# matteobutano/optimal_crowds

Hardware: NVIDIA B200
Metric: hjb_gcell_updates_per_s (higher is better)
Workload: dtype f64

## Files before the change

### optimal_crowds_b200/csrc/oc_hjb.cu

```cuda
#include <cmath>
#include <algorithm>
#include <vector>

#include "oc_common.h"
#include "oc_hjb_fused.cuh"
#include "oc_hjb_final.h"
#include "oc_rk45.h"
#include "oc_vels.h"

namespace {

constexpr int TX = 128, TY = 16, NTHREADS = 256;
constexpr int SW = TX + 2;

struct Comb {
    const double *y;
    const double *k[6];
    double a[6];
    double h;
};

template <int N>
__device__ __forceinline__ double comb_eval(const Comb &c, size_t idx) {
    if (N == 0) return c.y[idx];
// ... 233 lines not shown
    size_t pool_used = 0;
    cudaEvent_t get_event() {
        if (pool_used == pool.size()) { cudaEvent_t e; cudaEventCreate(&e); pool.push_back(e); }
        return pool[pool_used++];
    }
    void begin(int cls, double bytes) {
        if (!profile) return;
        Rec r{cls, bytes, get_event(), get_event()};
        cudaEventRecord(r.a, st);
        recs.push_back(r);
    }
    void end() {
        if (!profile) return;
        cudaEventRecord(recs.back().b, st);
    }
    void collect(oc_hjb_stats *out) {
        for (auto &r : recs) {
            float ms = 0;
            cudaEventElapsedTime(&ms, r.a, r.b);
            out->cls_launches[r.cls]++;
            out->cls_ms[r.cls] += ms;
            out->cls_bytes[r.cls] += r.bytes;
        }
        for (auto e : pool) cudaEventDestroy(e);
        pool.clear(); recs.clear();
    }

    template <int N, int MODE>
    void launch_stage(const Comb &c, double *kout, double *yn, const ErrArgs &ea) {
        dim3 grid(nbx, nby);
        begin(0, 8.0 * (double)n * (MODE == 1 ? 9 : N + 3));
        hjb_stage_kernel<N, MODE><<<grid, NTHREADS, 0, st>>>(c, coef, kout, yn, ea, partial, Ny, Nx, diff_over_dxdy);
        end();
        launches++;
    }
    void stage(int N, const Comb &c, double *kout) {
        ErrArgs ea{};
        switch (N) {
            case 0: launch_stage<0, 0>(c, kout, nullptr, ea); break;
            case 1: launch_stage<1, 0>(c, kout, nullptr, ea); break;
            case 2: launch_stage<2, 0>(c, kout, nullptr, ea); break;
            case 3: launch_stage<3, 0>(c, kout, nullptr, ea); break;
            case 4: launch_stage<4, 0>(c, kout, nullptr, ea); break;
            case 5: launch_stage<5, 0>(c, kout, nullptr, ea); break;
        }
    }
    int fused_rc = 0, fused_gx = 0, fused_gy = 0;
    void fused_plan(int n_sm, int forced_rc = 0) {
        fused_gx = (Nx + fused::VX - 1) / fused::VX;
        fused_rc = forced_rc > 0 ? forced_rc : fused::plan_chunk_rows(Nx, Ny, n_sm, 1, 0);
        fused_gy = (Ny + fused_rc - 1) / fused_rc;
    }
    fused::MapCache maps;
    int launch_fused(int ne, fused::Args &a) {
        fused::set_tensor_maps(a, Ny, &maps);
        dim3 grid(fused_gx, fused_gy);
        begin(0, 8.0 * (double)n * (5 + ne));
        OC_CUDA(fused::launch<false>(ne, a, grid, st));
        end();
        launches++;
        return OC_OK;
    }
    int reduce_to_host(size_t off, double *out, int gx = -1, int gy = -1) {
        if (gx < 0) { gx = nbx; gy = nby; }
        begin(2, 8.0 * ((double)gx * gy + gy));
        rowgroup_sum_kernel<<<gy, NTHREADS, 0, st>>>(partial + off, gx, rowsum_d);
        end();
        launches++;
        OC_CUDA(cudaMemcpyAsync(rowsum_h, rowsum_d, sizeof(double) * gy, cudaMemcpyDeviceToHost, st));
        OC_CUDA(cudaStreamSynchronize(st));
        double s = 0.0;
        for (int i = 0; i < gy; i++) s += rowsum_h[i];
        *out = s;
        return OC_OK;
    }
};

int ensure_ws(oc_ctx *ctx, size_t n, int nbx, int nby) {
    int rc = oc_ensure_buffer(ctx->hjb_ws, ctx->hjb_ws_bytes, 10 * n * sizeof(double), false, "HJB workspace");
    if (rc) return rc;
    size_t np = (size_t)2 * nbx * nby + nby + 64;
    {
        size_t fgx = (size_t)(nbx * TX + fused::VX - 1) / fused::VX + 1, fgy = (size_t)(nby * TY + 15) / 16 + 1;
        np = std::max(np, 2 * fgx * fgy + fgy + 64);
    }
    if ((rc = oc_ensure_buffer(ctx->hjb_partial, ctx->hjb_partial_bytes, np * sizeof(double), false, "HJB partial sums")))
        return rc;
    size_t hp = (size_t)std::max(nby, (nby * TY + 15) / 16 + 1) + 16;
    return oc_ensure_buffer(ctx->h_pinned, ctx->h_pinned_bytes, hp * sizeof(double), true, "pinned host scratch");
}

int ensure_final_reduce(oc_ctx *ctx, int slots) { return ocfinal::ensure(ctx, slots); }
void final_reduce_args(oc_ctx *ctx, int slot, fused::Args &fa) { ocfinal::set_args(ctx, slot, ++ctx->fr_seq, fa); }
inline bool final_ready(oc_ctx *ctx, int slot, unsigned long long seq, double *out) { return ocfinal::ready(ctx, slot, seq, out); }
int wait_final(oc_ctx *ctx, int slot, unsigned long long seq, cudaStream_t st, double *out) {
    return ocfinal::wait(ctx, slot, seq, st, out);
}

}

extern "C" int oc_hjb_rhs(oc_ctx *ctx, const double *d_phi, const double *d_V, const double *d_m,
                          const oc_hjb_params *prm, double *d_out, void *stream) {
    OC_ARG(ctx && d_phi && d_V && prm && d_out, "NULL argument");
    OC_CUDA(cudaSetDevice(ctx->device));
    Solver s{};
    s.ctx = ctx; s.st = (cudaStream_t)stream; s.Ny = ctx->Ny; s.Nx = ctx->Nx;
    s.n = (size_t)s.Ny * s.Nx;
    s.nbx = (s.Nx + TX - 1) / TX; s.nby = (s.Ny + TY - 1) / TY;
    int rc = ensure_ws(ctx, s.n, s.nbx, s.nby);
    if (rc) return rc;
    s.coef = ctx->hjb_ws;
// ... 55 lines not shown
    s.profile = prm->profile != 0;
    OC_CUDA(cudaEventRecord(ctx->ev0, s.st));

    prep_kernel<<<(unsigned)((n + 255) / 256), 256, 0, s.st>>>(d_V, d_m, prm->g, 1.0 / (prm->mu * s2), n, s.coef, s.y);
    s.launches++;
    rk45::Controller ctl(T, t_eval, nt);
    {
        Comb c{};
        c.y = s.y;
        s.stage(0, c, s.K[0]);
        stats->nfev++;
    }
    if (ctl.needs_initial_step()) {
        dim3 grid(s.nbx, s.nby);
        init_norm_kernel<<<grid, NTHREADS, 0, s.st>>>(s.y, s.K[0], nullptr, rtol, atol, s.Ny, s.Nx, s.partial, 0);
        s.launches++;
        double s0, s1, sq2;
        if ((rc = s.reduce_to_host(0, &s0))) return rc;
        if ((rc = s.reduce_to_host((size_t)s.nbx * s.nby, &s1))) return rc;
        const double d1 = std::sqrt(s1) / sqrt_n;
        const double h0 = ctl.initial_h0(std::sqrt(s0) / sqrt_n, d1);
        Comb c{};
        c.y = s.y; c.k[0] = s.K[0]; c.a[0] = 1.0; c.h = h0 * ctl.direction;
        s.stage(1, c, s.K[1]);
        stats->nfev++;
        init_norm_kernel<<<grid, NTHREADS, 0, s.st>>>(s.y, s.K[0], s.K[1], rtol, atol, s.Ny, s.Nx, s.partial, 1);
        s.launches++;
        if ((rc = s.reduce_to_host(0, &sq2))) return rc;
        ctl.set_initial_step(h0, d1, std::sqrt(sq2) / sqrt_n / h0);
    }
    stats->h0 = ctl.h_abs;

    bool use_fused = prm->fused != 0 && s.Ny > fused::HY + 1 && s.Nx > fused::HX + 1, fused_attempt = false;
    double *phi_scratch = nullptr;
    if (use_fused) {
        int n_sm = 148;
        cudaDeviceGetAttribute(&n_sm, cudaDevAttrMultiProcessorCount, ctx->device);
        s.fused_plan(n_sm, prm->chunk_rows);
        size_t np_need = (size_t)2 * s.fused_gx * s.fused_gy + s.fused_gy;
        if (ctx->hjb_partial_bytes < np_need * sizeof(double) || ctx->h_pinned_bytes < ((size_t)s.fused_gy + 16) * sizeof(double)) {
            oc::set_error("internal: fused partial buffers too small");
            return OC_ERR_ARG;
        }
        if (!d_phi && d_vx && d_vy) {
            size_t need = (size_t)fused::NE_MAX * n * sizeof(double);
            if ((rc = oc_ensure_buffer(ctx->hjb_scratch, ctx->hjb_scratch_bytes, need, false, "phi scratch"))) return rc;
            phi_scratch = ctx->hjb_scratch;
        }
    }
    const size_t n_int = (size_t)(s.Ny - 2) * (s.Nx - 2);
    const bool final_in_kernel = use_fused && s.fused_gy <= fused::MAX_FINAL_ROWS;
    if (final_in_kernel && (rc = ensure_final_reduce(ctx, 1))) return rc;
    const bool want_out = d_phi || (d_vx && d_vy);

    while (ctl.begin_step()) {
        bool accepted = false;
        while (!accepted && ctl.propose(prm->forced_h, prm->n_forced_h)) {
            const double h = ctl.h;
            fused_attempt = use_fused && (!want_out || d_phi || ctl.n_emit() <= fused::NE_MAX);
            double se;
            if (fused_attempt) {
                fused::Args fa{};
                fa.y = s.y; fa.k1 = s.K[0]; fa.coef = s.coef; fa.ynew = s.ynew; fa.k7 = s.K[6]; fa.partial = s.partial;
                fa.A = s.diff_over_dxdy; fa.rtol = rtol; fa.atol = atol;
                fa.Ny = s.Ny; fa.Nx = s.Nx; fa.RC = s.fused_rc;
                fa.row_base = 0; fa.own0 = 0; fa.own1 = s.Ny; fa.phi_row_base = 0;
                const int n_emit = want_out ? ctl.n_emit() : 0;
                int e0 = 0;
                do {
                    const int ne = std::min(n_emit - e0, fused::NE_MAX);
                    fused::set_attempt(fa, ctl, e0, ne, d_phi, phi_scratch, n);
                    if (final_in_kernel) final_reduce_args(ctx, 0, fa);
                    if ((rc = s.launch_fused(ne, fa))) return rc;
                    e0 += ne;
                } while (e0 < n_emit);
                stats->nfev += 6;
                if (final_in_kernel) {
                    if ((rc = wait_final(ctx, 0, fa.seq, s.st, &se))) return rc;
                } else if ((rc = s.reduce_to_host(0, &se, s.fused_gx, s.fused_gy))) return rc;
            } else {
            for (int sgi = 1; sgi < 6; sgi++) {
                Comb c{};
                c.y = s.y; c.h = h;
                for (int j = 0; j < sgi; j++) { c.k[j] = s.K[j]; c.a[j] = rk45::A[sgi][j]; }
                s.stage(sgi, c, s.K[sgi]);
            }
            {
                Comb c{};
                c.y = s.y; c.h = h;
                int m = 0;
                for (int j = 0; j < 6; j++)
                    if (j != 1) { c.k[m] = s.K[j]; c.a[m] = rk45::B[j]; m++; }
                ErrArgs ea{};
                for (int j = 0; j < 6; j++) ea.k[j] = s.K[j];
                for (int j = 0; j < 7; j++) ea.e[j] = rk45::E[j];
                ea.h = h; ea.rtol = rtol; ea.atol = atol;
                s.launch_stage<5, 1>(c, s.K[6], s.ynew, ea);
            }
            stats->nfev += 6;
            if ((rc = s.reduce_to_host(0, &se))) return rc;
            }
            const double error_norm = std::sqrt(se) / sqrt_n;
            const int ntr = ctl.attempts();
            if (trace_h && ntr < trace_cap) { trace_h[ntr] = h; trace_err[ntr] = error_norm; }
            accepted = ctl.judge(error_norm);
        }
        if (!accepted) break;

        if (fused_attempt) {
            for (int e = 0; e < ctl.n_emit(); e++) {
                const int kd = ctl.sample_column(e);
                if (d_vx && d_vy && kd >= 1) {
                    const double *ph = fused::sample_slice(ctl, e, d_phi, phi_scratch, n);
                    const int sl = nt - 1 - kd;
                    dim3 grid((s.Nx - 2 + 63) / 64, (s.Ny - 2 + 3) / 4);
                    s.begin(1, 8.0 * (double)n * 3);
                    vels_kernel<<<grid, NTHREADS, 0, s.st>>>(ph, s.Ny, s.Nx, prm->mu, prm->lim, 1.0 / (2 * ctx->dx), 1.0 / (2 * ctx->dy),
                                                             d_vx + (size_t)sl * n_int, d_vy + (size_t)sl * n_int);
                    s.end();
                    s.launches++;
                }
            }
        } else {
            int e = 0;
            while (e < ctl.n_emit()) {
                DenseArgs a{};
                a.yold = s.y;
                for (int j = 0; j < 7; j++) { a.k[j] = s.K[j]; for (int p = 0; p < 4; p++) a.P[j][p] = rk45::P[j][p]; }
                a.h = ctl.h; a.mu = prm->mu; a.lim = prm->lim; a.inv_two_dx = 1.0 / (2 * ctx->dx); a.inv_two_dy = 1.0 / (2 * ctx->dy);
                int m = 0;
                bool any = false;
                for (; m < DMAX && e < ctl.n_emit(); e++) {
                    int kd = ctl.sample_column(e);
                    a.x[m] = ctl.sample_x(e);
                    a.phi[m] = d_phi ? d_phi + (size_t)kd * n : nullptr;
                    int sl = nt - 1 - kd;
                    bool has_v = d_vx && d_vy && kd >= 1;
                    a.vx[m] = has_v ? d_vx + (size_t)sl * n_int : nullptr;
                    a.vy[m] = has_v ? d_vy + (size_t)sl * n_int : nullptr;
                    if (a.phi[m] || a.vx[m]) { any = true; m++; }
                }
                a.n_emit = m;
                if (any) {
                    dim3 grid((s.Nx + DTX - 1) / DTX, (s.Ny + DTY - 1) / DTY);
                    double words = 7.0;
                    for (int q = 0; q < m; q++) words += (a.phi[q] ? 1.0 : 0.0) + (a.vx[q] ? 2.0 : 0.0);
                    s.begin(1, 8.0 * (double)n * words);
                    hjb_dense_kernel<<<grid, NTHREADS, 0, s.st>>>(a, s.Ny, s.Nx);
                    s.end();
                    s.launches++;
                }
            }
        }
        ctl.accept();
        std::swap(s.y, s.ynew);
        std::swap(s.K[0], s.K[6]);
    }
    OC_CUDA(cudaEventRecord(ctx->ev1, s.st));
    OC_CUDA(cudaStreamSynchronize(s.st));
    OC_CUDA(cudaGetLastError());
    float ms = 0;
    OC_CUDA(cudaEventElapsedTime(&ms, ctx->ev0, ctx->ev1));
    stats->gpu_ms = ms;
    s.collect(stats);
    ctl.report(stats);
    stats->launches = s.launches;
    oc::count_launch(s.launches);
    if (trace_n) *trace_n = ctl.attempts();
    if (ctl.status == -1) {
        oc::set_error("RK45: required step size is less than spacing between numbers (t=%g)", ctl.t);
        return OC_ERR_STEP_TOO_SMALL;
    }
    return OC_OK;
}

namespace {

struct BatchRoom {
    Solver s;
    enum Phase { START, INIT0, INIT1, STEP, DONE } phase = START;
    const double *V = nullptr, *m = nullptr;
    double *phi = nullptr, *scratch = nullptr, *vx = nullptr, *vy = nullptr;
    double *rs_d = nullptr, *rs_h = nullptr;
    int rs_stride = 0;
    cudaEvent_t ev = nullptr;
    unsigned long long wait_seq = 0;
    rk45::Controller ctl;
    double g = 0, inv_mu_s2 = 0, mu = 0;
    double h0 = 0, d1 = 0;
    double step_sum = 0.0;
    fused::Args fa{};
    oc_hjb_stats st{};
};

}

extern "C" int oc_hjb_solve_batch(oc_ctx *ctx, int n_rooms, const double *const *d_V, const double *const *d_m,
                                  const oc_hjb_params *prm, double T, const double *t_eval, int nt,
                                  double *const *d_phi, double *const *d_vx, double *const *d_vy,
                                  oc_hjb_stats *stats, void *stream) {
    OC_ARG(prm && n_rooms >= 1, "NULL argument");
    std::vector<oc_hjb_room> same(n_rooms, oc_hjb_room{prm->sigma, prm->mu, prm->g, T, t_eval, nt, 0});
    return oc_hjb_solve_multi(ctx, n_rooms, d_V, d_m, same.data(), prm, d_phi, d_vx, d_vy, stats, stream);
}

extern "C" int oc_hjb_solve_multi(oc_ctx *ctx, int n_rooms, const double *const *d_V, const double *const *d_m,
                                  const oc_hjb_room *spec, const oc_hjb_params *prm, double *const *d_phi,
                                  double *const *d_vx, double *const *d_vy, oc_hjb_stats *stats, void *stream) {
    OC_ARG(ctx && d_V && prm && stats && n_rooms >= 1, "NULL argument");
// ... 281 lines not shown
```

### optimal_crowds_b200/csrc/oc_hjb_fused.cuh

```cuda
#pragma once
#include <cuda.h>
#include <cuda_runtime.h>

#include <cstddef>
#include <cstdint>

#include "oc_rk45.h"

namespace fused {

#ifndef OC_BX
#define OC_BX 128
#endif
#ifndef OC_PF
#define OC_PF 6
#endif
#ifndef OC_PD
#define OC_PD (OC_PF - 1)
#endif
constexpr int BX = OC_BX;
constexpr int HX = 8;
constexpr int VX = BX - 2 * HX;
constexpr int HY = 6;
constexpr int PF = OC_PF;
// ... 40 lines not shown
    double *phi[NE_MAX];
    double ha21;
    double ha3[2], ha4[3], ha5[4], ha6[5];
    double hb[6];
    double he[7];
    double w[NE_MAX][7];
    double A;
    double rtol, atol;
    int Ny, Nx, RC;
    int row_base, own0, own1, phi_row_base;
    unsigned *ticket;
    double *result;
    unsigned long long *result_seq;
    unsigned long long seq;
    double *peer_ynew[2], *peer_k7[2];
    int peer_row_base[2];
    int nranks, my_rank;
    double *peer_inbox[P2P_MAX_RANKS];
};
constexpr int MAX_FINAL_ROWS = 2 * 6 * (BX + 2) - 8;

inline double *sample_slice(const rk45::Controller &c, int e, double *phi, double *scratch, size_t slice) {
    return phi ? phi + (size_t)c.sample_column(e) * slice : scratch + (size_t)(e % NE_MAX) * slice;
}
inline void set_attempt(Args &a, const rk45::Controller &c, int e0, int ne, double *phi, double *scratch, size_t slice) {
    const double h = c.h;
    a.ha21 = h * rk45::A[1][0];
    for (int j = 0; j < 2; j++) a.ha3[j] = h * rk45::A[2][j];
    for (int j = 0; j < 3; j++) a.ha4[j] = h * rk45::A[3][j];
    for (int j = 0; j < 4; j++) a.ha5[j] = h * rk45::A[4][j];
    for (int j = 0; j < 5; j++) a.ha6[j] = h * rk45::A[5][j];
    for (int j = 0; j < 6; j++) a.hb[j] = h * rk45::B[j];
    for (int j = 0; j < 7; j++) a.he[j] = h * rk45::E[j];
    for (int i = 0; i < ne; i++) {
        const double x = c.sample_x(e0 + i);
        const double pw[4] = {x, x * x, x * x * x, x * x * x * x};
        for (int j = 0; j < 7; j++) {
            double acc = 0.0;
            for (int q = 0; q < 4; q++) acc += rk45::P[j][q] * pw[q];
            a.w[i][j] = h * acc;
        }
        a.phi[i] = sample_slice(c, e0 + i, phi, scratch, slice);
    }
}

__device__ __forceinline__ void cp_async8_if(void *smem, const void *gmem, bool ok) {
    unsigned s = (unsigned)__cvta_generic_to_shared(smem);
    asm volatile("{ .reg .pred p; setp.ne.b32 p, %2, 0; @p cp.async.ca.shared.global [%0], [%1], 8; }"
                 ::"r"(s), "l"(gmem), "r"((int)ok) : "memory");
}
__device__ __forceinline__ void st_if(double *p, double v, bool ok) {
    asm volatile("{ .reg .pred p; setp.ne.b32 p, %2, 0; @p st.global.f64 [%0], %1; }" ::"l"(p), "d"(v), "r"((int)ok) : "memory");
}
__device__ __forceinline__ void cp_async_commit() { asm volatile("cp.async.commit_group;" ::: "memory"); }
template <int N>
__device__ __forceinline__ void cp_async_wait() { asm volatile("cp.async.wait_group %0;" ::"n"(N) : "memory"); }

__device__ __forceinline__ void mbar_init(unsigned long long *bar, unsigned count) {
    asm volatile("mbarrier.init.shared::cta.b64 [%0], %1;" ::"r"((unsigned)__cvta_generic_to_shared(bar)), "r"(count) : "memory");
}
__device__ __forceinline__ void mbar_expect_tx(unsigned long long *bar, unsigned bytes) {
    asm volatile("mbarrier.arrive.expect_tx.shared::cta.b64 _, [%0], %1;"
                 ::"r"((unsigned)__cvta_generic_to_shared(bar)), "r"(bytes) : "memory");
}
__device__ __forceinline__ void bulk_g2s(void *smem, const void *gmem, unsigned bytes, unsigned long long *bar) {
    asm volatile("cp.async.bulk.shared::cluster.global.mbarrier::complete_tx::bytes [%0], [%1], %2, [%3];"
                 ::"r"((unsigned)__cvta_generic_to_shared(smem)), "l"(gmem), "r"(bytes),
                   "r"((unsigned)__cvta_generic_to_shared(bar)) : "memory");
}
__device__ __forceinline__ void tma_g2s_2d(unsigned smem, const CUtensorMap *map, int cx, int cy, unsigned bar) {
    asm volatile("cp.async.bulk.tensor.2d.shared::cluster.global.tile.mbarrier::complete_tx::bytes [%0], [%1, {%2, %3}], [%4];"
                 ::"r"(smem), "l"(reinterpret_cast<uint64_t>(map)), "r"(cx), "r"(cy), "r"(bar) : "memory");
}
__device__ __forceinline__ bool elect_one() {
    unsigned pred;
    asm volatile("{ .reg .pred p; elect.sync _|p, 0xffffffff; selp.u32 %0, 1, 0, p; }" : "=r"(pred));
    return pred != 0;
}
__device__ __forceinline__ void mbar_expect_tx_u32(unsigned bar, unsigned bytes) {
    asm volatile("mbarrier.arrive.expect_tx.shared::cta.b64 _, [%0], %1;" ::"r"(bar), "r"(bytes) : "memory");
}
__device__ __forceinline__ void bulk_g2s_u32(unsigned smem, const void *gmem, unsigned bytes, unsigned bar) {
    asm volatile("cp.async.bulk.shared::cluster.global.mbarrier::complete_tx::bytes [%0], [%1], %2, [%3];"
                 ::"r"(smem), "l"(gmem), "r"(bytes), "r"(bar) : "memory");
}
__device__ __forceinline__ void mbar_wait_u32(unsigned bar, unsigned parity) {
    asm volatile(
        "{\n"
        ".reg .pred p;\n"
        "OC_WAITU_%=:\n"
        "mbarrier.try_wait.parity.shared::cta.b64 p, [%0], %1;\n"
        "@p bra OC_DONEU_%=;\n"
        "bra OC_WAITU_%=;\n"
        "OC_DONEU_%=:\n"
        "}\n" ::"r"(bar), "r"(parity) : "memory");
}
__device__ __forceinline__ void mbar_wait(unsigned long long *bar, unsigned parity) {
    asm volatile(
        "{\n"
        ".reg .pred p;\n"
        "OC_WAIT_%=:\n"
        "mbarrier.try_wait.parity.shared::cta.b64 p, [%0], %1;\n"
        "@p bra OC_DONE_%=;\n"
        "bra OC_WAIT_%=;\n"
        "OC_DONE_%=:\n"
        "}\n" ::"r"((unsigned)__cvta_generic_to_shared(bar)), "r"(parity) : "memory");
}

__device__ __forceinline__ double rhs_pre(double up, double lf, double rt, double C, double Aw, double dw) {
    return fma(Aw, (up + lf) + rt, dw * C);
}
__device__ __forceinline__ double rhs_fin(double pre, double dn, double Aw) { return fma(Aw, dn, pre); }

__device__ __forceinline__ double rcp_pos(double x) {
    double r;
    asm("rcp.approx.ftz.f64 %0, %1;" : "=d"(r) : "d"(x));
    double e = fma(-x, r, 1.0);
    r = fma(r, e, r);
    e = fma(-x, r, 1.0);
    r = fma(r, e, r);
    return r;
}

struct __align__(128) Smem {
    double pf[NG][3][GR][BX];
    double2 ex[2][3][BX + 2];
    double cst[(1 + NE_MAX) * 6];
    double red[BX / 32];
    unsigned long long full[NG];
};
static_assert(sizeof(double2) * 2 * 3 * (BX + 2) >= sizeof(double) * MAX_FINAL_ROWS, "final reduction staging");

__device__ __forceinline__ int mirror(int i, int n) { return i < 0 ? -i : (i >= n ? 2 * (n - 1) - i : i); }

template <int NE, bool P2P, bool BULK>
__device__ __forceinline__ void hjb_fused_body(const Args &a) {
    extern __shared__ __align__(128) unsigned char smem_raw[];
    Smem &sm = *reinterpret_cast<Smem *>(smem_raw);
    const int tid = threadIdx.x;
    const int x0 = blockIdx.x * VX - HX;
    const int gx = x0 + tid;
    const int c0 = max(x0, 0), c1 = min(x0 + BX, a.Nx);
    const int gxm = min(max(mirror(gx, a.Nx), c0), c1 - 1);
    const int lt = BULK ? gxm - x0 : tid;
    const int y0 = a.own0 + blockIdx.y * a.RC;
    const int y1 = min(y0 + a.RC, a.own1);
    const bool col_out = tid >= HX && tid < BX - HX && gx < a.Nx;
    const int phi_shift = (a.row_base - a.phi_row_base) * a.Nx;

    for (int i = tid; i < 2 * 3 * (BX + 2); i += BX) (&sm.ex[0][0][0])[i] = make_double2(0.0, 0.0);
    if (tid < 6) {
        const int j = tid == 0 ? 0 : tid + 1;
        sm.cst[tid] = a.he[j];
#pragma unroll
        for (int ee = 0; ee < NE; ee++) sm.cst[6 * (ee + 1) + tid] = a.w[ee][j];
    }
    if (BULK && tid == 0) {
#pragma unroll
        for (int s = 0; s < NG; s++) mbar_init(&sm.full[s], 1);
        asm volatile("fence.mbarrier_init.release.cluster;" ::: "memory");
    }
    __syncthreads();
    unsigned sm_pf = (unsigned)__cvta_generic_to_shared(&sm.pf[0][0][0][0]);
    unsigned sm_full = (unsigned)__cvta_generic_to_shared(&sm.full[0]);
    asm volatile("" : "+r"(sm_pf), "+r"(sm_full));

    double yw[7], k1w[7], Aw[7], dw[7], k2w[5], k3w[7], k4w[7], k5w[7], k6w[7];
    double u2[3], u3[4], u4[5], u5[6], u6[7], un[8];
#pragma unroll
    for (int i = 0; i < 7; i++) { yw[i] = 0; k1w[i] = 0; Aw[i] = 0; dw[i] = 0; k3w[i] = 0; k4w[i] = 0; k5w[i] = 0; k6w[i] = 0; }
#pragma unroll
    for (int i = 0; i < 5; i++) k2w[i] = 0;
    u2[0] = u2[1] = u2[2] = 0; u3[1] = u3[2] = u3[3] = 0; u4[2] = u4[3] = u4[4] = 0;
    u5[3] = u5[4] = u5[5] = 0; u6[4] = u6[5] = u6[6] = 0; un[5] = un[6] = un[7] = 0;

    const int r_begin = y0 - HY, r_end = y1 + HY;
    const unsigned row_bytes = (unsigned)(c1 - c0) * 8u;
    const int warp = __shfl_sync(0xffffffffu, tid >> 5, 0);
    constexpr unsigned TILE_BYTES = 3u * GR * BX * 8u, FIELD_BYTES = GR * BX * 8u, ROW_BYTES = BX * 8u;
    auto issue_group = [&](int ga, int slot) {
        if (warp == 0 && ga < r_end && elect_one()) {
            const unsigned bar = sm_full + 8u * slot, dst = sm_pf + TILE_BYTES * slot;
            if (ga >= 0 && ga + GR <= a.Ny) {
                mbar_expect_tx_u32(bar, TILE_BYTES);
                tma_g2s_2d(dst, &a.tm_y, x0, ga - a.row_base, bar);
                tma_g2s_2d(dst + FIELD_BYTES, &a.tm_k1, x0, ga - a.row_base, bar);
                tma_g2s_2d(dst + 2u * FIELD_BYTES, &a.tm_coef, x0, ga - a.row_base, bar);
            } else {
                mbar_expect_tx_u32(bar, 3u * GR * row_bytes);
#pragma unroll 1
                for (int j = 0; j < GR; j++) {
                    const int rm = min(max(mirror(ga + j, a.Ny), 0), a.Ny - 1);
                    const int g = (rm - a.row_base) * a.Nx + c0;
                    const unsigned d = dst + ROW_BYTES * j + 8u * (c0 - x0);
                    bulk_g2s_u32(d, a.y + g, row_bytes, bar);
                    bulk_g2s_u32(d + FIELD_BYTES, a.k1 + g, row_bytes, bar);
                    bulk_g2s_u32(d + 2u * FIELD_BYTES, a.coef + g, row_bytes, bar);
                }
            }
        }
    };
    auto issue = [&](int row, int slot) {
        const int rm = min(max(mirror(row, a.Ny), 0), a.Ny - 1);
        const int g = (rm - a.row_base) * a.Nx + gxm;
        const bool ok = row < r_end;
        cp_async8_if(&sm.pf[0][0][slot][tid], a.y + g, ok);
        cp_async8_if(&sm.pf[0][1][slot][tid], a.k1 + g, ok);
        cp_async8_if(&sm.pf[0][2][slot][tid], a.coef + g, ok);
        cp_async_commit();
    };

    if (BULK) issue_group(r_begin, 0);
    else {
#pragma unroll 1
        for (int q = 0; q < PD; q++) issue(r_begin + q, q);
    }

    constexpr int NV = NE < OC_VREGCONST ? NE : OC_VREGCONST;
    double wv[NV > 0 ? NV : 1][6], hev[6];
#pragma unroll
    for (int ee = 0; ee < NV; ee++)
#pragma unroll
        for (int j = 0; j < 6; j++) wv[ee][j] = sm.cst[6 * (ee + 1) + j];
#pragma unroll
    for (int j = 0; j < 6; j++) hev[j] = a.he[j == 0 ? 0 : j + 1];
    const double dwall = -4.0 * a.A;

    double acc = 0.0;
    unsigned ph_base = 0;
#pragma unroll 1
    for (int rb = r_begin; rb < r_end; rb += UNROLL) {
#pragma unroll
      for (int uu = 0; uu < UNROLL; uu++) {
        const int r = rb + uu;
        const int s0 = uu % PF;
        const int buf = uu & 1;
        const int gi = uu / GR, gj = uu % GR;
        if (BULK) {
            if (gj == 0) {
                issue_group(r + GR, gi ^ 1);
                if (r < r_end) mbar_wait_u32(sm_full + 8u * gi, ph_base);
            }
        } else {
            issue(r + PD, (s0 + PD) % PF);
            cp_async_wait<PD>();
        }
        const double *ring = BULK ? &sm.pf[gi][0][gj][lt] : &sm.pf[0][0][s0][lt];
        yw[0] = ring[0];
        k1w[0] = ring[GR * BX];
        {
            const double cf = ring[2 * GR * BX];
            const bool wall = cf != cf;
            Aw[0] = wall ? 0.0 : a.A;
            dw[0] = wall ? 0.0 : dwall - cf;
        }
        const double2 *exp_ = &sm.ex[buf ^ 1][0][tid];
        double2 *exc = &sm.ex[buf][0][tid + 1];
#ifdef OC_ABL_NOEX
        const double2 l23 = make_double2(u2[1], u3[2]), r23 = l23, l45 = make_double2(u4[3], u5[4]), r45 = l45,
                      l6n = make_double2(u6[5], un[6]), r6n = l6n;
#else
        const double2 l23 = exp_[0], r23 = exp_[2];
        const double2 l45 = exp_[BX + 2], r45 = exp_[BX + 2 + 2];
        const double2 l6n = exp_[2 * (BX + 2)], r6n = exp_[2 * (BX + 2) + 2];
#endif
        const double p2 = rhs_pre(u2[2], l23.x, r23.x, u2[1], Aw[1], dw[1]);
        const double p3 = rhs_pre(u3[3], l23.y, r23.y, u3[2], Aw[2], dw[2]);
        const double p4 = rhs_pre(u4[4], l45.x, r45.x, u4[3], Aw[3], dw[3]);
        const double p5 = rhs_pre(u5[5], l45.y, r45.y, u5[4], Aw[4], dw[4]);
        const double p6 = rhs_pre(u6[6], l6n.x, r6n.x, u6[5], Aw[5], dw[5]);
        const double p7 = rhs_pre(un[7], l6n.y, r6n.y, un[6], Aw[6], dw[6]);
        const double q3 = fma(a.ha3[0], k1w[1], yw[1]);
        const double q4 = fma(a.ha4[1], k2w[2], fma(a.ha4[0], k1w[2], yw[2]));
        const double q5 = fma(a.ha5[2], k3w[3], fma(a.ha5[1], k2w[3], fma(a.ha5[0], k1w[3], yw[3])));
        const double q6 = fma(a.ha6[3], k4w[4], fma(a.ha6[2], k3w[4], fma(a.ha6[1], k2w[4], fma(a.ha6[0], k1w[4], yw[4]))));
        const double qn = fma(a.hb[4], k5w[5], fma(a.hb[3], k4w[5], fma(a.hb[2], k3w[5], fma(a.hb[0], k1w[5], yw[5]))));
        u2[0] = fma(a.ha21, k1w[0], yw[0]);
#ifdef OC_CHAIN1
        k2w[1] = rhs_fin(p2, u2[0], Aw[1]);
        k3w[2] = fma(Aw[2] * a.ha3[1], k2w[1], fma(Aw[2], q3, p3));
        k4w[3] = fma(Aw[3] * a.ha4[2], k3w[2], fma(Aw[3], q4, p4));
        k5w[4] = fma(Aw[4] * a.ha5[3], k4w[3], fma(Aw[4], q5, p5));
        k6w[5] = fma(Aw[5] * a.ha6[4], k5w[4], fma(Aw[5], q6, p6));
        u3[1] = fma(a.ha3[1], k2w[1], q3);
        u4[2] = fma(a.ha4[2], k3w[2], q4);
        u5[3] = fma(a.ha5[3], k4w[3], q5);
        u6[4] = fma(a.ha6[4], k5w[4], q6);
        un[5] = fma(a.hb[5], k6w[5], qn);
        const double k7 = fma(Aw[6] * a.hb[5], k6w[5], fma(Aw[6], qn, p7));
#else
        k2w[1] = rhs_fin(p2, u2[0], Aw[1]);
        u3[1] = fma(a.ha3[1], k2w[1], q3);
        k3w[2] = rhs_fin(p3, u3[1], Aw[2]);
        u4[2] = fma(a.ha4[2], k3w[2], q4);
        k4w[3] = rhs_fin(p4, u4[2], Aw[3]);
        u5[3] = fma(a.ha5[3], k4w[3], q5);
        k5w[4] = rhs_fin(p5, u5[3], Aw[4]);
        u6[4] = fma(a.ha6[4], k5w[4], q6);
        k6w[5] = rhs_fin(p6, u6[4], Aw[5]);
        un[5] = fma(a.hb[5], k6w[5], qn);
        const double k7 = rhs_fin(p7, un[5], Aw[6]);
#endif
#ifndef OC_ABL_NOEX
        exc[0] = make_double2(u2[0], u3[1]);
        exc[BX + 2] = make_double2(u4[2], u5[3]);
        exc[2 * (BX + 2)] = make_double2(u6[4], un[5]);
#endif
        {
            const int row = r - 6;
#ifdef OC_ABL_NOSTORE
            const bool ok = col_out && row >= y0 && row < y1 && a.Nx < 0;
#else
            const bool ok = col_out && row >= y0 && row < y1;
#endif
            const int g = (row - a.row_base) * a.Nx + gx;
            double e = fma(hev[5], k7, fma(hev[4], k6w[6], fma(hev[3], k5w[6], fma(hev[2], k4w[6], fma(hev[1], k3w[6], hev[0] * k1w[6])))));
            double sc = fma(fmax(fabs(yw[6]), fabs(un[6])), a.rtol, a.atol);
            double qq = e * rcp_pos(sc);
            acc = ok ? fma(qq, qq, acc) : acc;
            st_if(a.ynew + g, un[6], ok);
            st_if(a.k7 + g, k7, ok);
#pragma unroll
            for (int ee = 0; ee < NE; ee++) {
                double ph;
#ifdef OC_ABL_NOPHI
                if (true) ph = k7; else
#endif
                if (ee < NV)
                    ph = fma(wv[ee][5], k7, fma(wv[ee][4], k6w[6], fma(wv[ee][3], k5w[6], fma(wv[ee][2], k4w[6],
                             fma(wv[ee][1], k3w[6], fma(wv[ee][0], k1w[6], yw[6]))))));
                else
                    ph = fma(a.w[ee][6], k7, fma(a.w[ee][5], k6w[6], fma(a.w[ee][4], k5w[6],
                             fma(a.w[ee][3], k4w[6], fma(a.w[ee][2], k3w[6], fma(a.w[ee][0], k1w[6], yw[6]))))));
                st_if(a.phi[ee] + (g + phi_shift), ph, ok);
            }
        }
#ifndef OC_ABL_NOSYNC
        __syncthreads();
#endif
#pragma unroll
        for (int l = 6; l > 0; l--) { yw[l] = yw[l - 1]; k1w[l] = k1w[l - 1]; Aw[l] = Aw[l - 1]; dw[l] = dw[l - 1]; }
        k2w[4] = k2w[3]; k2w[3] = k2w[2]; k2w[2] = k2w[1];
        k3w[6] = k3w[5]; k3w[5] = k3w[4]; k3w[4] = k3w[3]; k3w[3] = k3w[2];
        k4w[6] = k4w[5]; k4w[5] = k4w[4]; k4w[4] = k4w[3];
        k5w[6] = k5w[5]; k5w[5] = k5w[4];
        k6w[6] = k6w[5];
        u2[2] = u2[1]; u2[1] = u2[0];
        u3[3] = u3[2]; u3[2] = u3[1];
        u4[4] = u4[3]; u4[3] = u4[2];
        u5[5] = u5[4]; u5[4] = u5[3];
        u6[6] = u6[5]; u6[5] = u6[4];
        un[7] = un[6]; un[6] = un[5];
      }
      ph_base ^= 1u;
    }
    if (!BULK) cp_async_wait<0>();
    if (P2P && col_out) {
        if (y0 == a.own0 && a.peer_ynew[0] != nullptr)
            for (int row = a.own0; row < min(a.own0 + HY, y1); row++) {
                const int g = (row - a.row_base) * a.Nx + gx, gp = (row - a.peer_row_base[0]) * a.Nx + gx;
                a.peer_ynew[0][gp] = a.ynew[g];
                a.peer_k7[0][gp] = a.k7[g];
            }
        if (y1 == a.own1 && a.peer_ynew[1] != nullptr)
            for (int row = max(a.own1 - HY, y0); row < a.own1; row++) {
                const int g = (row - a.row_base) * a.Nx + gx, gp = (row - a.peer_row_base[1]) * a.Nx + gx;
                a.peer_ynew[1][gp] = a.ynew[g];
                a.peer_k7[1][gp] = a.k7[g];
            }
    }
#pragma unroll
    for (int o = 16; o > 0; o >>= 1) acc += __shfl_down_sync(0xffffffffu, acc, o);
    if ((tid & 31) == 0) sm.red[tid >> 5] = acc;
    __syncthreads();
    if (tid == 0) {
        double s = 0.0;
#pragma unroll
        for (int i = 0; i < BX / 32; i++) s += sm.red[i];
        a.partial[(size_t)blockIdx.y * gridDim.x + blockIdx.x] = s;
    }
    if (a.ticket == nullptr) return;
    __shared__ int is_last;
    if (tid == 0) {
        if (P2P) __threadfence_system();
        else __threadfence();
        const unsigned t = atomicAdd(a.ticket, 1u);
        is_last = (t == gridDim.x * gridDim.y - 1);
    }
    __syncthreads();
    if (!is_last) return;
    __threadfence();
    double *rows = reinterpret_cast<double *>(&sm.ex[0][0][0]);
    const int ngx = gridDim.x, gy = gridDim.y, lane = tid & 31;
    for (int row = tid >> 5; row < gy; row += BX / 32) {
// ... 6 lines not shown
        double srow = 0.0;
#pragma unroll
        for (int vw = 0; vw < 8; vw++) {
#pragma unroll
            for (int o = 16; o > 0; o >>= 1) v[vw] += __shfl_down_sync(0xffffffffu, v[vw], o);
            srow += v[vw];
        }
        if (lane == 0) rows[row] = srow;
    }
    __syncthreads();
    if (P2P) {
        const int par = (int)(a.seq & 1ull);
        if (tid < a.nranks) {
            double *dst = a.peer_inbox[tid] + (size_t)(par * P2P_MAX_RANKS + a.my_rank) * P2P_INBOX_STRIDE;
            for (int r = 0; r < gy; r++) *reinterpret_cast<volatile double *>(dst + r) = rows[r];
            __threadfence_system();
            *reinterpret_cast<volatile unsigned long long *>(dst + P2P_INBOX_STRIDE - 1) = a.seq;
            const volatile unsigned long long *flag = reinterpret_cast<const volatile unsigned long long *>(
                a.peer_inbox[a.my_rank] + (size_t)(par * P2P_MAX_RANKS + tid) * P2P_INBOX_STRIDE + P2P_INBOX_STRIDE - 1);
            long long it = 0;
            while (*flag != a.seq) {
                if (++it > 40000000ll) { is_last = 2; break; }
                __nanosleep(200);
            }
            __threadfence_system();
        }
        __syncthreads();
        if (tid == 0 && is_last == 2) {
            *a.ticket = 0u;
            *reinterpret_cast<volatile unsigned long long *>(a.result_seq) = a.seq | (1ull << 63);
        } else if (tid == 0) {
            double tot = 0.0;
            for (int q = 0; q < a.nranks; q++) {
                const volatile double *src = a.peer_inbox[a.my_rank] + (size_t)(par * P2P_MAX_RANKS + q) * P2P_INBOX_STRIDE;
                for (int r = 0; r < gy; r++) tot += src[r];
            }
            *a.ticket = 0u;
            *reinterpret_cast<volatile double *>(a.result) = tot;
            __threadfence_system();
            *reinterpret_cast<volatile unsigned long long *>(a.result_seq) = a.seq;
        }
        return;
    }
    if (tid == 0) {
        double tot = 0.0;
        for (int r = 0; r < gy; r++) tot += rows[r];
        *a.ticket = 0u;
        *reinterpret_cast<volatile double *>(a.result) = tot;
        __threadfence_system();
        *reinterpret_cast<volatile unsigned long long *>(a.result_seq) = a.seq;
    }
}

template <int NE, bool P2P = false, bool BULK = true>
__global__ void __launch_bounds__(BX, CTAS_PER_SM) hjb_fused_kernel(const __grid_constant__ Args a) {
    hjb_fused_body<NE, P2P, BULK>(a);
}

constexpr int BATCH_MAX = 24;
struct BatchArgs {
    Args a[BATCH_MAX];
};
static_assert(sizeof(BatchArgs) <= 32764, "kernel parameter space");
template <int NE, bool BULK>
__global__ void __launch_bounds__(BX, CTAS_PER_SM) hjb_fused_batch_kernel(const __grid_constant__ BatchArgs ba) {
    hjb_fused_body<NE, false, BULK>(ba.a[blockIdx.z]);
}

inline bool bulk_ok(const Args &a) {
#ifdef OC_NO_BULK
    return false;
#else
    return a.tma != 0 && (a.Nx % 2 == 0) && (((uintptr_t)a.y | (uintptr_t)a.k1 | (uintptr_t)a.coef) % 16 == 0);
#endif
}

inline bool make_tensor_map(CUtensorMap *tm, const double *base, int rows, int Nx) {
    typedef CUresult (*encode_fn)(CUtensorMap *, CUtensorMapDataType, cuuint32_t, void *, const cuuint64_t *, const cuuint64_t *,
                                  const cuuint32_t *, const cuuint32_t *, CUtensorMapInterleave, CUtensorMapSwizzle,
                                  CUtensorMapL2promotion, CUtensorMapFloatOOBfill);
    static encode_fn encode = nullptr;
    static bool tried = false;
    if (!tried) {
        tried = true;
        void *fn = nullptr;
        cudaDriverEntryPointQueryResult qres;
        if (cudaGetDriverEntryPoint("cuTensorMapEncodeTiled", &fn, cudaEnableDefault, &qres) == cudaSuccess &&
            qres == cudaDriverEntryPointSuccess)
            encode = reinterpret_cast<encode_fn>(fn);
        else
            cudaGetLastError();
    }
    if (!encode || Nx % 2 != 0 || ((uintptr_t)base % 16) != 0) return false;
    const cuuint64_t dims[2] = {(cuuint64_t)Nx, (cuuint64_t)rows};
    const cuuint64_t strides[1] = {(cuuint64_t)Nx * sizeof(double)};
    const cuuint32_t box[2] = {(cuuint32_t)BX, (cuuint32_t)GR};
    const cuuint32_t estr[2] = {1, 1};
    return encode(tm, CU_TENSOR_MAP_DATA_TYPE_FLOAT64, 2, const_cast<double *>(base), dims, strides, box, estr,
                  CU_TENSOR_MAP_INTERLEAVE_NONE, CU_TENSOR_MAP_SWIZZLE_NONE, CU_TENSOR_MAP_L2_PROMOTION_L2_128B,
                  CU_TENSOR_MAP_FLOAT_OOB_FILL_NONE) == CUDA_SUCCESS;
}
struct MapCache {
    static constexpr int CAP = 8;
    const double *base[CAP];
    int rows[CAP], n = 0;
    CUtensorMap tm[CAP];
    bool get(const double *b, int r, int Nx, CUtensorMap *out) {
        for (int i = 0; i < n; i++)
            if (base[i] == b && rows[i] == r) { *out = tm[i]; return true; }
        CUtensorMap t;
        if (!make_tensor_map(&t, b, r, Nx)) return false;
        if (n < CAP) { base[n] = b; rows[n] = r; tm[n] = t; n++; }
        *out = t;
        return true;
    }
};
inline void set_tensor_maps(Args &a, int rows, MapCache *cache = nullptr) {
    MapCache local;
    MapCache &c = cache ? *cache : local;
    a.tma = c.get(a.y, rows, a.Nx, &a.tm_y) && c.get(a.k1, rows, a.Nx, &a.tm_k1) && c.get(a.coef, rows, a.Nx, &a.tm_coef);
}
template <int NE, bool P2P, bool BULK>
inline cudaError_t launch_one(const Args &a, dim3 grid, cudaStream_t st) {
    if (sizeof(Smem) > 48 * 1024) {
        cudaError_t e = cudaFuncSetAttribute(hjb_fused_kernel<NE, P2P, BULK>, cudaFuncAttributeMaxDynamicSharedMemorySize,
                                             (int)sizeof(Smem));
        if (e != cudaSuccess) return e;
    }
    hjb_fused_kernel<NE, P2P, BULK><<<grid, BX, sizeof(Smem), st>>>(a);
    return cudaSuccess;
}
template <bool P2P>
inline cudaError_t launch(int ne, const Args &a, dim3 grid, cudaStream_t st) {
    const bool bulk = bulk_ok(a);
#define OC_FUSED_CASE(NE) \
    case NE: return bulk ? launch_one<NE, P2P, true>(a, grid, st) : launch_one<NE, P2P, false>(a, grid, st);
    switch (ne) {
        OC_FUSED_CASE(0) OC_FUSED_CASE(1) OC_FUSED_CASE(2) OC_FUSED_CASE(3) OC_FUSED_CASE(4) OC_FUSED_CASE(5)
        default: return bulk ? launch_one<6, P2P, true>(a, grid, st) : launch_one<6, P2P, false>(a, grid, st);
    }
#undef OC_FUSED_CASE
}

template <int NE, bool BULK>
inline cudaError_t launch_batch_one(const BatchArgs &ba, dim3 grid, cudaStream_t st) {
    if (sizeof(Smem) > 48 * 1024) {
        cudaError_t e = cudaFuncSetAttribute(hjb_fused_batch_kernel<NE, BULK>, cudaFuncAttributeMaxDynamicSharedMemorySize,
                                             (int)sizeof(Smem));
        if (e != cudaSuccess) return e;
    }
    hjb_fused_batch_kernel<NE, BULK><<<grid, BX, sizeof(Smem), st>>>(ba);
    return cudaSuccess;
}
inline cudaError_t launch_batch(int ne, const BatchArgs &ba, int nb, dim3 grid2d, cudaStream_t st) {
    bool bulk = true;
    for (int q = 0; q < nb; q++) bulk = bulk && bulk_ok(ba.a[q]);
    const dim3 grid(grid2d.x, grid2d.y, nb);
#define OC_FUSED_CASE(NE) \
    case NE: return bulk ? launch_batch_one<NE, true>(ba, grid, st) : launch_batch_one<NE, false>(ba, grid, st);
    switch (ne) {
        OC_FUSED_CASE(0) OC_FUSED_CASE(1) OC_FUSED_CASE(2) OC_FUSED_CASE(3) OC_FUSED_CASE(4) OC_FUSED_CASE(5)
        default: return bulk ? launch_batch_one<6, true>(ba, grid, st) : launch_batch_one<6, false>(ba, grid, st);
    }
#undef OC_FUSED_CASE
}

}
```

Measured before the change: 459.3.

## Recompute first RK stage in fused HJB kernel instead of streaming k1/k7

Adds a REC variant of the fused RK45 kernel. After an accepted fused step it recomputes k1 (the FSAL stage) from y and coef inside the kernel rather than loading it from global memory, and it writes k7 only at boundary cells. It loads one extra y row per tile and fetches k1 only for edge rows and columns via bulk copies, which removes two full-field streams per step. The cost is extra stencil arithmetic, more complex TMA expect-tx bookkeeping and a larger shared tile layout, with risk of subtle boundary mismatches.

```diff
diff --git a/optimal_crowds_b200/csrc/oc_hjb.cu b/optimal_crowds_b200/csrc/oc_hjb.cu
--- a/optimal_crowds_b200/csrc/oc_hjb.cu
+++ b/optimal_crowds_b200/csrc/oc_hjb.cu
@@ -309,11 +309,11 @@
         fused_gy = (Ny + fused_rc - 1) / fused_rc;
     }
     fused::MapCache maps;
-    int launch_fused(int ne, fused::Args &a) {
-        fused::set_tensor_maps(a, Ny, &maps);
+    int launch_fused(int ne, fused::Args &a, bool rec = false) {
+        fused::set_tensor_maps(a, Ny, &maps, rec);
         dim3 grid(fused_gx, fused_gy);
-        begin(0, 8.0 * (double)n * (5 + ne));
-        OC_CUDA(fused::launch<false>(ne, a, grid, st));
+        begin(0, 8.0 * (double)n * ((rec ? 3 : 5) + ne));
+        OC_CUDA((rec ? fused::launch<false, true>(ne, a, grid, st) : fused::launch<false>(ne, a, grid, st)));
         end();
         launches++;
         return OC_OK;
@@ -475,6 +475,7 @@
     const bool final_in_kernel = use_fused && s.fused_gy <= fused::MAX_FINAL_ROWS;
     if (final_in_kernel && (rc = ensure_final_reduce(ctx, 1))) return rc;
     const bool want_out = d_phi || (d_vx && d_vy);
+    bool rec_f = false;
 
     while (ctl.begin_step()) {
         bool accepted = false;
@@ -494,7 +495,7 @@
                     const int ne = std::min(n_emit - e0, fused::NE_MAX);
                     fused::set_attempt(fa, ctl, e0, ne, d_phi, phi_scratch, n);
                     if (final_in_kernel) final_reduce_args(ctx, 0, fa);
-                    if ((rc = s.launch_fused(ne, fa))) return rc;
+                    if ((rc = s.launch_fused(ne, fa, rec_f))) return rc;
                     e0 += ne;
                 } while (e0 < n_emit);
                 stats->nfev += 6;
@@ -578,6 +579,7 @@
         ctl.accept();
         std::swap(s.y, s.ynew);
         std::swap(s.K[0], s.K[6]);
+        rec_f = fused_attempt && d_phi;
     }
     OC_CUDA(cudaEventRecord(ctx->ev1, s.st));
     OC_CUDA(cudaStreamSynchronize(s.st));
diff --git a/optimal_crowds_b200/csrc/oc_hjb_fused.cuh b/optimal_crowds_b200/csrc/oc_hjb_fused.cuh
--- a/optimal_crowds_b200/csrc/oc_hjb_fused.cuh
+++ b/optimal_crowds_b200/csrc/oc_hjb_fused.cuh
@@ -116,6 +116,10 @@
 __device__ __forceinline__ void st_if(double *p, double v, bool ok) {
     asm volatile("{ .reg .pred p; setp.ne.b32 p, %2, 0; @p st.global.f64 [%0], %1; }" ::"l"(p), "d"(v), "r"((int)ok) : "memory");
 }
+__device__ __forceinline__ void lds_if(double &v, const double *p, bool ok) {
+    asm volatile("{ .reg .pred p; setp.ne.b32 p, %2, 0; @p ld.shared.f64 %0, [%1]; }"
+                 : "+d"(v) : "r"((unsigned)__cvta_generic_to_shared(p)), "r"((int)ok));
+}
 __device__ __forceinline__ void cp_async_commit() { asm volatile("cp.async.commit_group;" ::: "memory"); }
 template <int N>
 __device__ __forceinline__ void cp_async_wait() { asm volatile("cp.async.wait_group %0;" ::"n"(N) : "memory"); }
@@ -143,6 +147,9 @@
 }
 __device__ __forceinline__ void mbar_expect_tx_u32(unsigned bar, unsigned bytes) {
     asm volatile("mbarrier.arrive.expect_tx.shared::cta.b64 _, [%0], %1;" ::"r"(bar), "r"(bytes) : "memory");
+}
+__device__ __forceinline__ void mbar_add_tx_u32(unsigned bar, unsigned bytes) {
+    asm volatile("mbarrier.expect_tx.relaxed.cta.shared::cta.b64 [%0], %1;" ::"r"(bar), "r"(bytes) : "memory");
 }
 __device__ __forceinline__ void bulk_g2s_u32(unsigned smem, const void *gmem, unsigned bytes, unsigned bar) {
     asm volatile("cp.async.bulk.shared::cluster.global.mbarrier::complete_tx::bytes [%0], [%1], %2, [%3];"
@@ -186,8 +193,9 @@
     return r;
 }
 
+constexpr int TY_ = 0, TK1 = GR + 1, TCF = 2 * GR + 1, TROWS = 3 * GR + 1;
 struct __align__(128) Smem {
-    double pf[NG][3][GR][BX];
+    double pf[NG][TROWS][BX];
     double2 ex[2][3][BX + 2];
     double cst[(1 + NE_MAX) * 6];
     double red[BX / 32];
@@ -197,8 +205,9 @@
 
 __device__ __forceinline__ int mirror(int i, int n) { return i < 0 ? -i : (i >= n ? 2 * (n - 1) - i : i); }
 
-template <int NE, bool P2P, bool BULK>
+template <int NE, bool P2P, bool BULK, bool REC>
 __device__ __forceinline__ void hjb_fused_body(const Args &a) {
+    static_assert(!(REC && P2P), "the row-band solve streams f");
     extern __shared__ __align__(128) unsigned char smem_raw[];
     Smem &sm = *reinterpret_cast<Smem *>(smem_raw);
     const int tid = threadIdx.x;
@@ -225,7 +234,7 @@
         asm volatile("fence.mbarrier_init.release.cluster;" ::: "memory");
     }
     __syncthreads();
-    unsigned sm_pf = (unsigned)__cvta_generic_to_shared(&sm.pf[0][0][0][0]);
+    unsigned sm_pf = (unsigned)__cvta_generic_to_shared(&sm.pf[0][0][0]);
     unsigned sm_full = (unsigned)__cvta_generic_to_shared(&sm.full[0]);
     asm volatile("" : "+r"(sm_pf), "+r"(sm_full));
 
@@ -241,25 +250,53 @@
     const int r_begin = y0 - HY, r_end = y1 + HY;
     const unsigned row_bytes = (unsigned)(c1 - c0) * 8u;
     const int warp = __shfl_sync(0xffffffffu, tid >> 5, 0);
-    constexpr unsigned TILE_BYTES = 3u * GR * BX * 8u, FIELD_BYTES = GR * BX * 8u, ROW_BYTES = BX * 8u;
+    constexpr unsigned TILE_BYTES = TROWS * BX * 8u, ROW_BYTES = BX * 8u;
+    constexpr unsigned K1_OFF = TK1 * ROW_BYTES, CF_OFF = TCF * ROW_BYTES;
+    const bool col_mirrored = gx < 0 || gx >= a.Nx;
+    const int il = min(max(BULK ? lt - 1 : (col_mirrored ? tid + 1 : tid - 1), 0), BX - 1);
+    const int ir = min(max(BULK ? lt + 1 : (col_mirrored ? tid - 1 : tid + 1), 0), BX - 1);
+    const bool col_edge = gxm == 0 || gxm == a.Nx - 1;
+    auto edge = [&](int row) { return col_edge || row == 0 || row == a.Ny - 1; };
     auto issue_group = [&](int ga, int slot) {
         if (warp == 0 && ga < r_end && elect_one()) {
             const unsigned bar = sm_full + 8u * slot, dst = sm_pf + TILE_BYTES * slot;
-            if (ga >= 0 && ga + GR <= a.Ny) {
-                mbar_expect_tx_u32(bar, TILE_BYTES);
-                tma_g2s_2d(dst, &a.tm_y, x0, ga - a.row_base, bar);
-                tma_g2s_2d(dst + FIELD_BYTES, &a.tm_k1, x0, ga - a.row_base, bar);
-                tma_g2s_2d(dst + 2u * FIELD_BYTES, &a.tm_coef, x0, ga - a.row_base, bar);
-            } else {
-                mbar_expect_tx_u32(bar, 3u * GR * row_bytes);
+            if (REC) {
 #pragma unroll 1
                 for (int j = 0; j < GR; j++) {
+                    const int rm = min(max(mirror(ga + j, a.Ny), 0), a.Ny - 1);
+                    const double *src = a.k1 + (rm - a.row_base) * a.Nx;
+                    const unsigned d = dst + K1_OFF + ROW_BYTES * j;
+                    if (rm == 0 || rm == a.Ny - 1) {
+                        mbar_add_tx_u32(bar, row_bytes);
+                        bulk_g2s_u32(d + 8u * (c0 - x0), src + c0, row_bytes, bar);
+                        continue;
+                    }
+                    if (x0 < 0) {
+                        mbar_add_tx_u32(bar, 16u);
+                        bulk_g2s_u32(d + 8u * (0 - x0), src, 16u, bar);
+                    }
+                    if (c1 == a.Nx) {
+                        mbar_add_tx_u32(bar, 16u);
+                        bulk_g2s_u32(d + 8u * (a.Nx - 2 - x0), src + a.Nx - 2, 16u, bar);
+                    }
+                }
+            }
+            if (ga >= 0 && ga + (REC ? GR + 1 : GR) <= a.Ny) {
+                mbar_expect_tx_u32(bar, REC ? (2 * GR + 1) * ROW_BYTES : 3u * GR * ROW_BYTES);
+                tma_g2s_2d(dst, &a.tm_y, x0, ga - a.row_base, bar);
+                if (!REC) tma_g2s_2d(dst + K1_OFF, &a.tm_k1, x0, ga - a.row_base, bar);
+                tma_g2s_2d(dst + CF_OFF, &a.tm_coef, x0, ga - a.row_base, bar);
+            } else {
+                mbar_expect_tx_u32(bar, (REC ? 2u * GR + 1u : 3u * GR) * row_bytes);
+#pragma unroll 1
+                for (int j = 0; j < (REC ? GR + 1 : GR); j++) {
                     const int rm = min(max(mirror(ga + j, a.Ny), 0), a.Ny - 1);
                     const int g = (rm - a.row_base) * a.Nx + c0;
                     const unsigned d = dst + ROW_BYTES * j + 8u * (c0 - x0);
                     bulk_g2s_u32(d, a.y + g, row_bytes, bar);
-                    bulk_g2s_u32(d + FIELD_BYTES, a.k1 + g, row_bytes, bar);
-                    bulk_g2s_u32(d + 2u * FIELD_BYTES, a.coef + g, row_bytes, bar);
+                    if (j == GR) break;
+                    if (!REC) bulk_g2s_u32(d + K1_OFF, a.k1 + g, row_bytes, bar);
+                    bulk_g2s_u32(d + CF_OFF, a.coef + g, row_bytes, bar);
                 }
             }
         }
@@ -267,17 +304,22 @@
     auto issue = [&](int row, int slot) {
         const int rm = min(max(mirror(row, a.Ny), 0), a.Ny - 1);
         const int g = (rm - a.row_base) * a.Nx + gxm;
-        const bool ok = row < r_end;
-        cp_async8_if(&sm.pf[0][0][slot][tid], a.y + g, ok);
-        cp_async8_if(&sm.pf[0][1][slot][tid], a.k1 + g, ok);
-        cp_async8_if(&sm.pf[0][2][slot][tid], a.coef + g, ok);
+        const bool ok = row < (REC ? r_end + 1 : r_end);
+        cp_async8_if(&sm.pf[0][TY_ + slot][tid], a.y + g, ok);
+        cp_async8_if(&sm.pf[0][TK1 + slot][tid], a.k1 + g, ok && (!REC || edge(row)));
+        cp_async8_if(&sm.pf[0][TCF + slot][tid], a.coef + g, ok);
         cp_async_commit();
     };
+    constexpr int LDG_WAIT = REC ? PD - 2 : PD;
 
     if (BULK) issue_group(r_begin, 0);
     else {
 #pragma unroll 1
         for (int q = 0; q < PD; q++) issue(r_begin + q, q);
+        if (REC) {
+            cp_async_wait<LDG_WAIT>();
+            __syncthreads();
+        }
     }
 
     constexpr int NV = NE < OC_VREGCONST ? NE : OC_VREGCONST;
@@ -289,6 +331,12 @@
 #pragma unroll
     for (int j = 0; j < 6; j++) hev[j] = a.he[j == 0 ? 0 : j + 1];
     const double dwall = -4.0 * a.A;
+
+    if (REC) {
+        auto y_at = [&](int row) { return a.y[(min(max(mirror(row, a.Ny), 0), a.Ny - 1) - a.row_base) * a.Nx + gxm]; };
+        yw[1] = y_at(r_begin - 1);
+        yw[0] = y_at(r_begin);
+    }
 
     double acc = 0.0;
     unsigned ph_base = 0;
@@ -307,16 +355,30 @@
             }
         } else {
             issue(r + PD, (s0 + PD) % PF);
-            cp_async_wait<PD>();
-        }
-        const double *ring = BULK ? &sm.pf[gi][0][gj][lt] : &sm.pf[0][0][s0][lt];
-        yw[0] = ring[0];
-        k1w[0] = ring[GR * BX];
+            cp_async_wait<LDG_WAIT>();
+        }
+        const double *row_y = BULK ? &sm.pf[gi][TY_ + gj][0] : &sm.pf[0][TY_ + s0][0];
+        const double *row_k1 = BULK ? &sm.pf[gi][TK1 + gj][0] : &sm.pf[0][TK1 + s0][0];
+        const double *row_cf = BULK ? &sm.pf[gi][TCF + gj][0] : &sm.pf[0][TCF + s0][0];
+        if (!REC) {
+            yw[0] = row_y[lt];
+            k1w[0] = row_k1[lt];
+        }
         {
-            const double cf = ring[2 * GR * BX];
+            const double cf = row_cf[lt];
             const bool wall = cf != cf;
             Aw[0] = wall ? 0.0 : a.A;
             dw[0] = wall ? 0.0 : dwall - cf;
+        }
+        double y_dn = 0.0;
+        if (REC) {
+            y_dn = (BULK ? row_y + BX : &sm.pf[0][TY_ + (s0 + 1) % PF][0])[lt];
+            const double lf = row_y[il], rt = row_y[ir];
+            const bool ghost = r < 0 || r >= a.Ny;
+            const double up = ghost ? y_dn : yw[1], dn = ghost ? yw[1] : y_dn;
+            double k1 = rhs_fin(rhs_pre(up, lf, rt, yw[0], Aw[0], dw[0]), dn, Aw[0]);
+            lds_if(k1, row_k1 + lt, edge(r));
+            k1w[0] = k1;
         }
         const double2 *exp_ = &sm.ex[buf ^ 1][0][tid];
         double2 *exc = &sm.ex[buf][0][tid + 1];
@@ -383,7 +445,7 @@
             double qq = e * rcp_pos(sc);
             acc = ok ? fma(qq, qq, acc) : acc;
             st_if(a.ynew + g, un[6], ok);
-            st_if(a.k7 + g, k7, ok);
+            st_if(a.k7 + g, k7, ok && (!REC || edge(row)));
 #pragma unroll
             for (int ee = 0; ee < NE; ee++) {
                 double ph;
@@ -404,6 +466,7 @@
 #endif
 #pragma unroll
         for (int l = 6; l > 0; l--) { yw[l] = yw[l - 1]; k1w[l] = k1w[l - 1]; Aw[l] = Aw[l - 1]; dw[l] = dw[l - 1]; }
+        if (REC) yw[0] = y_dn;
         k2w[4] = k2w[3]; k2w[3] = k2w[2]; k2w[2] = k2w[1];
         k3w[6] = k3w[5]; k3w[5] = k3w[4]; k3w[4] = k3w[3]; k3w[3] = k3w[2];
         k4w[6] = k4w[5]; k4w[5] = k4w[4]; k4w[4] = k4w[3];
@@ -516,9 +579,9 @@
     }
 }
 
-template <int NE, bool P2P = false, bool BULK = true>
+template <int NE, bool P2P = false, bool BULK = true, bool REC = false>
 __global__ void __launch_bounds__(BX, CTAS_PER_SM) hjb_fused_kernel(const __grid_constant__ Args a) {
-    hjb_fused_body<NE, P2P, BULK>(a);
+    hjb_fused_body<NE, P2P, BULK, REC>(a);
 }
 
 constexpr int BATCH_MAX = 24;
@@ -528,7 +591,7 @@
 static_assert(sizeof(BatchArgs) <= 32764, "kernel parameter space");
 template <int NE, bool BULK>
 __global__ void __launch_bounds__(BX, CTAS_PER_SM) hjb_fused_batch_kernel(const __grid_constant__ BatchArgs ba) {
-    hjb_fused_body<NE, false, BULK>(ba.a[blockIdx.z]);
+    hjb_fused_body<NE, false, BULK, false>(ba.a[blockIdx.z]);
 }
 
 inline bool bulk_ok(const Args &a) {
@@ -539,7 +602,7 @@
 #endif
 }
 
-inline bool make_tensor_map(CUtensorMap *tm, const double *base, int rows, int Nx) {
+inline bool make_tensor_map(CUtensorMap *tm, const double *base, int rows, int Nx, int box_rows) {
     typedef CUresult (*encode_fn)(CUtensorMap *, CUtensorMapDataType, cuuint32_t, void *, const cuuint64_t *, const cuuint64_t *,
                                   const cuuint32_t *, const cuuint32_t *, CUtensorMapInterleave, CUtensorMapSwizzle,
                                   CUtensorMapL2promotion, CUtensorMapFloatOOBfill);
@@ -558,7 +621,7 @@
     if (!encode || Nx % 2 != 0 || ((uintptr_t)base % 16) != 0) return false;
     const cuuint64_t dims[2] = {(cuuint64_t)Nx, (cuuint64_t)rows};
     const cuuint64_t strides[1] = {(cuuint64_t)Nx * sizeof(double)};
-    const cuuint32_t box[2] = {(cuuint32_t)BX, (cuuint32_t)GR};
+    const cuuint32_t box[2] = {(cuuint32_t)BX, (cuuint32_t)box_rows};
     const cuuint32_t estr[2] = {1, 1};
     return encode(tm, CU_TENSOR_MAP_DATA_TYPE_FLOAT64, 2, const_cast<double *>(base), dims, strides, box, estr,
                   CU_TENSOR_MAP_INTERLEAVE_NONE, CU_TENSOR_MAP_SWIZZLE_NONE, CU_TENSOR_MAP_L2_PROMOTION_L2_128B,
@@ -567,41 +630,42 @@
 struct MapCache {
     static constexpr int CAP = 8;
     const double *base[CAP];
-    int rows[CAP], n = 0;
+    int rows[CAP], box[CAP], n = 0;
     CUtensorMap tm[CAP];
-    bool get(const double *b, int r, int Nx, CUtensorMap *out) {
+    bool get(const double *b, int r, int Nx, int bx, CUtensorMap *out) {
         for (int i = 0; i < n; i++)
-            if (base[i] == b && rows[i] == r) { *out = tm[i]; return true; }
+            if (base[i] == b && rows[i] == r && box[i] == bx) { *out = tm[i]; return true; }
         CUtensorMap t;
-        if (!make_tensor_map(&t, b, r, Nx)) return false;
-        if (n < CAP) { base[n] = b; rows[n] = r; tm[n] = t; n++; }
+        if (!make_tensor_map(&t, b, r, Nx, bx)) return false;
+        if (n < CAP) { base[n] = b; rows[n] = r; box[n] = bx; tm[n] = t; n++; }
         *out = t;
         return true;
     }
 };
-inline void set_tensor_maps(Args &a, int rows, MapCache *cache = nullptr) {
+inline void set_tensor_maps(Args &a, int rows, MapCache *cache = nullptr, bool rec = false) {
     MapCache local;
     MapCache &c = cache ? *cache : local;
-    a.tma = c.get(a.y, rows, a.Nx, &a.tm_y) && c.get(a.k1, rows, a.Nx, &a.tm_k1) && c.get(a.coef, rows, a.Nx, &a.tm_coef);
-}
-template <int NE, bool P2P, bool BULK>
+    a.tma = c.get(a.y, rows, a.Nx, rec ? GR + 1 : GR, &a.tm_y) && (rec || c.get(a.k1, rows, a.Nx, GR, &a.tm_k1)) &&
+            c.get(a.coef, rows, a.Nx, GR, &a.tm_coef);
+}
+template <int NE, bool P2P, bool BULK, bool REC>
 inline cudaError_t launch_one(const Args &a, dim3 grid, cudaStream_t st) {
     if (sizeof(Smem) > 48 * 1024) {
-        cudaError_t e = cudaFuncSetAttribute(hjb_fused_kernel<NE, P2P, BULK>, cudaFuncAttributeMaxDynamicSharedMemorySize,
+        cudaError_t e = cudaFuncSetAttribute(hjb_fused_kernel<NE, P2P, BULK, REC>, cudaFuncAttributeMaxDynamicSharedMemorySize,
                                              (int)sizeof(Smem));
         if (e != cudaSuccess) return e;
     }
-    hjb_fused_kernel<NE, P2P, BULK><<<grid, BX, sizeof(Smem), st>>>(a);
+    hjb_fused_kernel<NE, P2P, BULK, REC><<<grid, BX, sizeof(Smem), st>>>(a);
     return cudaSuccess;
 }
-template <bool P2P>
+template <bool P2P, bool REC = false>
 inline cudaError_t launch(int ne, const Args &a, dim3 grid, cudaStream_t st) {
     const bool bulk = bulk_ok(a);
 #define OC_FUSED_CASE(NE) \
-    case NE: return bulk ? launch_one<NE, P2P, true>(a, grid, st) : launch_one<NE, P2P, false>(a, grid, st);
+    case NE: return bulk ? launch_one<NE, P2P, true, REC>(a, grid, st) : launch_one<NE, P2P, false, REC>(a, grid, st);
     switch (ne) {
         OC_FUSED_CASE(0) OC_FUSED_CASE(1) OC_FUSED_CASE(2) OC_FUSED_CASE(3) OC_FUSED_CASE(4) OC_FUSED_CASE(5)
-        default: return bulk ? launch_one<6, P2P, true>(a, grid, st) : launch_one<6, P2P, false>(a, grid, st);
+        default: return bulk ? launch_one<6, P2P, true, REC>(a, grid, st) : launch_one<6, P2P, false, REC>(a, grid, st);
     }
 #undef OC_FUSED_CASE
 }
```

New measurement: 416.5 (median of 6 runs). -9.3%, worse.
